# lh3/yak

Measured on AMD Instinct MI355X. Metric: distinct k-mers counted/sec (k=31), yak count -b37 two-pass protocol, .yak bit-exact, higher is better.
Workload: dtype u64

## Files before the change

### yak_amd/csrc/engine_ctx.cpp

```cpp
#include "engine_int.h"
#include <atomic>

static thread_local char g_err[512] = "";

extern "C" const char *yakamd_last_error(void) { return g_err; }
int yk_set_error(const char *fmt, ...) { va_list ap; va_start(ap, fmt); vsnprintf(g_err, sizeof(g_err), fmt, ap); va_end(ap); fprintf(stderr, "[E::yak_amd] %s\n", g_err); return -1; }

extern "C" int yakamd_device_count(void)
{
	int n = 0;
	if (hipGetDeviceCount(&n) != hipSuccess) return 0;
	int ok = 0;
	for (int i = 0; i < n; ++i) {
		hipDeviceProp_t pr;
		if (hipGetDeviceProperties(&pr, i) == hipSuccess && strncmp(pr.gcnArchName, "gfx950", 6) == 0) ++ok;
	}
	return ok;
}

extern "C" yakamd_ctx *yakamd_ctx_of(yak_ch_t *h) { return ctx_of(h); }

BloomView bloom_view(yakamd_ctx *c)
{
	BloomView b;
// ... 218 lines not shown
u64 yk_ctx_keys_total(yakamd_ctx *c) { return c->img_keys_total; }
void yk_ctx_range(yakamd_ctx *c, int *lo, int *hi) { *lo = c->plo; *hi = c->phi; }

struct yak_ht_t { uint32_t bits, count; uint32_t *used; uint64_t *keys; };

static std::atomic<int64_t> g_host_syncs{0};
extern "C" int64_t yakamd_host_syncs(void) { return g_host_syncs.load(); }

int yk_ctx_sync_host(yakamd_ctx *c, yak_ch_t *h)
{
	if (__atomic_load_n(&c->host_valid, __ATOMIC_ACQUIRE)) return 0;
	static std::mutex mu;
	std::lock_guard<std::mutex> lk(mu);
	if (c->host_valid) return 0;
	HIPCK(hipSetDevice(c->dev));
	++g_host_syncs;
	if (c->hm_slots < c->n_slots) {
		c->hm_keys.reset(); c->hm_used.reset(); c->hm_slots = 0;
		void *hk = 0, *hu = 0;
		HIPCK(hipHostMalloc(&hk, c->n_slots * 8));
		c->hm_keys.reset((u64*)hk);
		HIPCK(hipHostMalloc(&hu, c->n_slots / 8));
		c->hm_used.reset((u32*)hu);
		c->hm_slots = c->n_slots;
	}
	HIPCK(hipMemcpyAsync(c->hm_keys.get(), c->d_keys, c->n_slots * 8, hipMemcpyDeviceToHost, c->st));
	HIPCK(hipMemcpyAsync(c->hm_used.get(), c->d_used, c->n_slots / 8, hipMemcpyDeviceToHost, c->st));
	HIPCK(hipStreamSynchronize(c->st));
	if (!c->hts) c->hts.reset((yak_ht_t*)calloc(c->P, sizeof(yak_ht_t)));
	for (int p = 0; p < c->P; ++p) {
// ... 42 lines not shown
```

### yak_amd/csrc/engine_int.h

```cpp
#ifndef YK_ENGINE_INT_H
#define YK_ENGINE_INT_H
#include <stdio.h>
#include <stdlib.h>
#include <string.h>
#include <stdarg.h>
#include <vector>
#include <map>
#include <string>
#include <mutex>
#include <algorithm>
#include <memory>
#include "yk_device.h"
#include "tally.h"
#include "engine.h"
#include "dev_buf.h"

#define fail(...) yk_set_error(__VA_ARGS__)
#define HIPCK(x) do { hipError_t e_ = (x); if (e_ != hipSuccess) return fail("%s:%d: %s -> %s", __FILE__, __LINE__, #x, hipGetErrorString(e_)); } while (0)

static inline double now_ms() { return yk_now_ms(); }

static inline int64_t env_i64(const char *name, int64_t dflt) { return yk_knob(name, dflt); }

static inline int ceil_log2_u64(u64 x) { int b = 0; while ((1ull << b) < x) ++b; return b; }
// ... 26 lines not shown
struct HostFree { void operator()(void *p) const { (void)hipHostFree(p); } };
struct CFree { void operator()(void *p) const { free(p); } };
struct yak_ht_t;

struct Kept { DevBuf<Rec> own; Rec *d_rec = 0; u64 n = 0; u64 t0 = 0, span = 0; std::vector<u64> bstart; int fmt = 0; };

struct PassBufs {
	std::vector<Kept> kept; u64 kept_bytes = 0;
	AccTab acc = {}; DevBuf<AccSlot> acc_mem; u64 acc_count = 0;
	DevVec<Rec> rec;
	DevVec<uint8_t> hpc;
	DevVec<u64> newlist, miss, cand;
};

struct Retained { DevBuf<Rec> rec; u64 n = 0; std::vector<u64> bstart; };
struct Ret2 { DevBuf<Rec> r2; DevBuf<u64> sbstart, koff, kkc, segbase; DevBuf<u32> kc2; FastParams fp = {}; u64 n_total = 0, n_keys = 0; bool valid = false; };
struct RetainedInput { std::vector<Retained> l1; u64 l1_bytes = 0; Ret2 l2; };

struct yakamd_ctx {
	CtxStream st;
	int k = 0, pre = 0, P = 0, n_hash = 0, bf_shift = 0, nb = 0;
	bool has_bloom = false;
	int dev = 0, plo = 0, phi = 0;

	DevBuf<u32> d_bits, d_used, d_delta;
	DevBuf<u64> d_off, d_keys;
	u64 n_slots = 0;
	std::vector<u32> h_bits, h_count;
	std::vector<u64> h_off;
	u64 img_keys_total = 0;

	DevBuf<u32> d_bf; size_t bf_words = 0;
	bool bf_virgin = false;
	bool bf_deferred = false;
	DevBuf<u32> d_multi; int multi_bits = 0;

	bool delta_dirty = false;
	bool in_pass = false; int create_new = 0; bool bloom_mode = false; bool gate_off = false; int or_mode = 0;
	PassBufs pass;
	DevBuf<u64> d_counters, d_lastput, d_lpbatch;
	DevBuf<u32> d_missing, d_nmissing;
	DevVec<uint8_t> stage;
	bool hpc = false;
	DevVec<u32> rows; DevBuf<u64> d_partial, d_bstart; int nb_bits = 0;
	bool fast = false; u64 fast_budget = 0; u64 t_pass0 = 0; bool t_pass0_set = false; u64 keys_at_begin = 0;
// ... 11 lines not shown

	bool host_valid = false;
	std::unique_ptr<u64[], HostFree> hm_keys; std::unique_ptr<u32[], HostFree> hm_used; u64 hm_slots = 0;
	std::unique_ptr<yak_ht_t[], CFree> hts;
};

struct yak_ch_ext { yak_ch_t pub; yakamd_ctx *ctx; u32 magic; int n_sub; yak_ch_t **sub; };
#define EXT_MAGIC 0x59414b41u

static inline yakamd_ctx *ctx_of(const yak_ch_t *h)
{
	const yak_ch_ext *e = (const yak_ch_ext*)h;
	return (h && e->magic == EXT_MAGIC) ? e->ctx : 0;
}

static inline ImgView img_view(yakamd_ctx *c)
{
	ImgView v;
	v.bits = c->d_bits; v.off = c->d_off; v.keys = c->d_keys; v.used = c->d_used; v.delta = c->d_delta;
	v.pre = c->pre; v.k = c->k;
	return v;
}

struct ImageState { yakamd_ctx *c; bool sharded, in_pass; };
ImageState yk_image_state(const yak_ch_t *h);
yakamd_ctx *yk_whole_image_ctx(const yak_ch_t *h, int min_cnt, const char *what, const char *no_gpu, const char *even_k);

struct OutFile {
	FILE *f = 0;
	const char *name = "-";
	bool own = false;
	OutFile() = default;
	OutFile(const OutFile&) = delete;
	OutFile &operator=(const OutFile&) = delete;
	~OutFile() { if (own && f) fclose(f); }
	bool open(const char *fn) { own = fn && strcmp(fn, "-") != 0; if (own) name = fn; f = own ? fopen(fn, "wb") : stdout; return f != 0; }
// ... 37 lines not shown
```

### yak_amd/csrc/engine_pass.cpp

```cpp
#include "engine_int.h"
#include "seg_sort_tile.h"

static int acc_reserve(yakamd_ctx *c, u64 incoming)
{
	PassBufs &ps = c->pass;
	const u64 need = ps.acc_count + incoming;
	int want = std::max(c->pre + 2, ceil_log2_u64((u64)(need / 0.6) + 1));
	if (want < 12) want = 12;
	if (ps.acc.s && ps.acc.bits >= want) return 0;
	AccTab nt;
	DevBuf<AccSlot> mem;
	nt.bits = want; nt.pre = c->pre; nt.mask = (1ull << want) - 1;
	if (mem.alloc((size_t)1 << want)) return -1;
	nt.s = mem;
	yk_launch_acc_init(nt.s, 1ull << want, c->st);
	if (ps.acc.s) {
		yk_launch_acc_rehash(ps.acc, nt, c->st);
		HIPCK(hipStreamSynchronize(c->st));
	}
	ps.acc_mem = std::move(mem);
	ps.acc = nt;
	return 0;
}

// ... 192 lines not shown
		if (env_i64("YAKAMD_VERBOSE", 0)) fprintf(stderr, "[yak_amd] key-owning count: 2^%d slots per range (up to 2^%d ranges per sub-table), %u keys of LDS room, %zu B of LDS, %u boundary-crossing instances%s\n",
		                                          rng_log, rb, kmax, lds, xn[0], xn[1] ? " (list overflow: second sweep)" : "");
		if (hipStreamSynchronize(c->st) != hipSuccess) r = fail("count sweep failed");
	}
	return r;
}

int consume_records(yakamd_ctx *c, const Rec *d_rec, int64_t n_rec, u64 t0, u64 batch_lo, u64 batch_hi, const u64 *d_bstart, int hash_only, int ytag)
{
	if (n_rec <= 0) return 0;
	ImgView img = img_view(c);
	c->st_cur.n_instances += n_rec;
	if (batch_hi > c->t_end) c->t_end = batch_hi;
	if (!c->create_new) {
		c->delta_dirty = true;
		EvTimer tm(c->st);
		if (d_bstart) {
			const int r = count_own(c, d_rec, d_bstart, hash_only, ytag);
			if (r <= 0 || ytag) {
				insert_ms(c, tm);
				return r;
			}
		}
		const size_t lds = d_bstart ? count_lds_bytes(c) : 0;
		if (!lds && d_bstart && hash_only && c->nb_bits == c->pre && env_i64("YAKAMD_COUNT_RNG", 1) != 0) {
			const int r = count_by_ranges(c, d_rec, n_rec, d_bstart);
			if (r <= 0) {
				insert_ms(c, tm);
				return r;
			}
// ... 248 lines not shown
	const size_t NB = (size_t)1 << c->nb_bits;
	if (part_reserve(c, 1)) return -1;
	HIPCK(hipMemcpyAsync(c->d_bstart, h_bstart, (NB + 1) * 8, hipMemcpyHostToDevice, c->st));
	const int r = consume_records(c, (const Rec*)d_hash_u64, n, 0, 0, 0, c->d_bstart, 1);
	HIPCK(hipStreamSynchronize(c->st));
	return r;
}

extern "C" int yakamd_count_hashes_dev(yak_ch_t *h, const void *d_hash_u64, int64_t n)
{
	yakamd_ctx *c = ctx_of(h);
	if (!c || !c->in_pass || c->create_new) return fail("count_hashes needs an open create_new = 0 pass");
	HIPCK(hipSetDevice(c->dev));
	if (n <= 0) return 0;
	c->delta_dirty = true;
	EvTimer tm(c->st);
	yk_launch_img_count_h((const u64*)d_hash_u64, n, img_view(c), c->st);
	insert_ms(c, tm);
	c->st_cur.n_instances += n;
	return 0;
}

extern "C" int yakamd_retain_input(yak_ch_t *h, int on)
{
	yakamd_ctx *c = ctx_of(h);
	if (!c) return fail("not an engine table");
	if (c->in_pass) return fail("yakamd_retain_input inside a pass");
	HIPCK(hipSetDevice(c->dev));
	c->retain_on = on != 0;
	if (!on) retained_drop(c);
// ... 4 lines not shown
{
	yakamd_ctx *c = ctx_of(h);
	if (!c || c->retain_broken) return 0;
	u64 n = c->ret.l2.valid ? c->ret.l2.n_total : 0;
	for (auto &r : c->ret.l1) n += r.n;
	return (int64_t)n;
}

extern "C" int yakamd_count_retained(yak_ch_t *h)
{
	yakamd_ctx *c = ctx_of(h);
	if (!c || !c->in_pass || c->create_new) return fail("yakamd_count_retained needs an open create_new = 0 pass");
	HIPCK(hipSetDevice(c->dev));
	const Ret2 &l2 = c->ret.l2;
	if (l2.valid && !c->retain_broken && l2.kc2) {
		EvTimer tm(c->st);
		yk_launch_cnt2_apply(l2.fp, l2.kkc, l2.kc2, l2.segbase, img_view(c), c->st);
		const double ms = insert_ms(c, tm);
		const bool bad = hipGetLastError() != hipSuccess;
		c->st_cur.n_instances += (int64_t)l2.n_total;
		c->st_cur.pass2_path = 1; yk_event(YKE_PASS2_FUSED);
		if (env_i64("YAKAMD_VERBOSE", 0)) fprintf(stderr, "[yak_amd] count pass: the counts of the pass before applied (%llu keys, %.2f ms)\n", (unsigned long long)l2.n_keys, ms);
		retained_drop(c);
		return bad ? fail("applying the counts of the pass before failed") : 0;
	}
	if (l2.valid && !c->retain_broken) {
		DevBuf<u32> d_kcnt;
		if (d_kcnt.alloc(l2.n_keys)) return -1;
		HIPCK(hipMemsetAsync(c->d_nmissing, 0, 4, c->st));
		EvTimer tm(c->st);
		yk_launch_cnt2(l2.fp, l2.sbstart, l2.r2, l2.koff, l2.kkc, l2.segbase, d_kcnt, img_view(c), l2.n_keys, c->d_nmissing, c->st);
		u32 used = 1;
		(void)hipMemcpyAsync(&used, c->d_nmissing, 4, hipMemcpyDeviceToHost, c->st);
		const double ms = insert_ms(c, tm);
		if (used) c->delta_dirty = true;
		d_kcnt.reset();
		const bool bad = hipGetLastError() != hipSuccess;
// ... 127 lines not shown
```

### yak_amd/csrc/engine_slice.cpp

```cpp
#include "engine_int.h"
#include "seg_sort_tile.h"

void chunk_runs(ChunkTable &t, const void *base, size_t stride, const u64 *start, size_t n_buckets, u64 len)
{
	t.h.clear();
	t.first.assign(n_buckets + 1, 0);
	for (size_t q = 0; q < n_buckets; ++q) {
		t.first[q] = (u32)t.h.size();
		for (u64 o = start[q]; o < start[q + 1]; o += len) {
			Chunk2 ch = {};
			ch.rec = (const Rec*)((const char*)base + o * stride); ch.n = (u32)std::min<u64>(len, start[q + 1] - o); ch.bucket = (u32)q;
			t.h.push_back(ch);
		}
		if (t.h.size() > t.first[q]) t.h.back().spare = 1;
	}
	t.first[n_buckets] = (u32)t.h.size();
}


struct Slice {
	FastParams fp;
	u64 n_total = 0, sort_tmax = 0, budget = 0;
	int fmt_in = 0, s2 = 0, s2a = 0, s2b = 0;
	bool three = false, nowb_plan = false, keep2 = false;
// ... 376 lines not shown
	s.r2.reset(); s.ovf2.reset();
	if (slice_gather(c, s)) return -1;
	s.lo_kc.reset(); s.lo_T.reset(); s.lo_nsel.reset(); s.lo_lp.reset(); s.lo_nd.reset(); s.lo_c2.reset();
	s.kc2.reset(); s.sbstart.reset(); s.ndist.reset(); s.koff.reset();
	s.lap(c, "gather of the selected keys");
	if (slice_sort(c, s)) return -1;
	s.kc[s.cur ^ 1].reset(); s.tt[s.cur ^ 1].reset();
	s.lap(c, "sort by insertion time");
	{
		EvTimer tm(c->st);
		s.ro.resize(c->P);
		if (yk_run_replay(c, s.m, s.kc[s.cur], s.tt[s.cur], c->d_lastput, 0, false, &s.ro)) return -1;
		c->st_cur.ms_replay += tm.stop();
	}
	s.lap(c, "exact layout");
	return 0;
}

int fast_abandon(yakamd_ctx *c)
{
	for (auto &k : c->pass.kept) if (k.fmt) return fail("a batch was fed out of stream order after tagged 8-byte batches were kept: feed in order, or set YAKAMD_REC8=0");
	c->fast = false;
	yk_event(YKE_FAST_ABANDONED);
	c->retain_broken = true; retained_drop(c);
	int r = 0;
	for (auto &k : c->pass.kept) {
		if (!r) r = consume_records(c, k.d_rec, (int64_t)k.n, k.t0, k.t0, k.t0 + k.span);
		k.own.reset();
	}
	c->pass.kept.clear(); c->pass.kept_bytes = 0;
// ... 53 lines not shown
```

### yak_amd/csrc/engine_table.cpp

```cpp
#include "engine_int.h"

int yk_ctx_hist(yakamd_ctx *c, int64_t *cnt1024)
{
	HIPCK(hipSetDevice(c->dev));
	DevBuf<u64> d_h;
	if (d_h.alloc(1024)) return -1;
	HIPCK(hipMemsetAsync(d_h, 0, 1024 * 8, c->st));
	yk_launch_img_hist(img_view(c), c->n_slots, d_h, c->st);
	const hipError_t e = hipMemcpyAsync(cnt1024, d_h, 1024 * 8, hipMemcpyDeviceToHost, c->st);
	const hipError_t e2 = hipStreamSynchronize(c->st);
	return e == hipSuccess && e2 == hipSuccess ? 0 : fail("hist: %s", hipGetErrorString(e != hipSuccess ? e : e2));
}

int yk_ctx_setcnt(yakamd_ctx *c, int cnt)
{
	HIPCK(hipSetDevice(c->dev));
	yk_launch_img_setcnt(img_view(c), c->n_slots, (u32)cnt & 1023u, c->st);
	HIPCK(hipStreamSynchronize(c->st));
	c->host_valid = false;
	return 0;
}

int yk_ctx_clear(yakamd_ctx *c)
{
	HIPCK(hipSetDevice(c->dev));
	yk_launch_img_clear(img_view(c), c->n_slots, c->st);
	HIPCK(hipStreamSynchronize(c->st));
	c->host_valid = false;
	return 0;
}

static int rebuild(yakamd_ctx *c, int cmin, int cmax, int which, yakamd_ctx *other, u64 *tot)
{
	HIPCK(hipSetDevice(c->dev));
	const int P = c->P;
	if (other && (other->pre != c->pre || other->k != c->k)) return fail("tables of different k / prefix length");
	const ImgView ov = other ? img_view(other) : img_view(c);
	std::vector<u32> m(P), init(P);
	std::vector<u64> seg_off(P + 1, 0);
	DevBuf<u64> d_kc, d_segoff; DevBuf<u32> d_segcnt;
	const int RG = yk_shrink_shares();
	std::vector<u32> mr((size_t)P * RG);
	if (d_segcnt.alloc((size_t)P * RG) || d_segoff.alloc(P + 1)) return -1;
	yk_launch_shrink_count(img_view(c), P, cmin, cmax, which, ov, d_segcnt, c->st, 1);
// ... 11 lines not shown
	const int r = yk_run_replay(c, m, d_kc, 0, 0, &init, true);
	c->st_last.ms_shrink = tm.stop();
	if (r) return r;
	*tot = c->img_keys_total;
	return 0;
}

int yk_ctx_shrink(yakamd_ctx *c, int cmin, int cmax, u64 *tot) { return rebuild(c, cmin, cmax, 0, 0, tot); }
int yk_ctx_subtract(yakamd_ctx *c, yakamd_ctx *other, u64 *tot) { return rebuild(c, 0, 1023, 1, other, tot); }
int yk_ctx_isec(yakamd_ctx *c, yakamd_ctx *other, u64 *tot) { return rebuild(c, 0, 1023, 2, other, tot); }

#define YK_LEAVE 0xfffffffeu
static int resize_tables(yakamd_ctx *c, const std::vector<u32> &new_bits)
{
	HIPCK(hipSetDevice(c->dev));
	const int P = c->P;
	std::vector<ResizeTask> tasks(P);
	std::vector<u64> new_off(P);
	std::vector<u32> bits_after(P);
	u64 tot = 0;
	for (int p = 0; p < P; ++p) {
		ResizeTask &t = tasks[p];
		t.old_bits = c->h_bits[p]; t.old_off = c->h_off[p]; t.pad = 0;
		t.rehash = new_bits[p] != YK_LEAVE;
		t.new_bits = t.rehash ? new_bits[p] : c->h_bits[p];
		bits_after[p] = t.new_bits;
		const u64 n = t.old_bits == YK_NOCAP ? 0 : (u64)1 << t.old_bits, N = t.new_bits == YK_NOCAP ? 0 : (u64)1 << t.new_bits;
		t.new_off = new_off[p] = tot;
		tot += std::max<u64>(32, std::max(n, N));
	}
// ... 63 lines not shown
	HIPCK(hipStreamSynchronize(c->st));
	*d_hash = hash.release(); *d_t = t.release();
	if (d_cnt) *d_cnt = cnt.release();
	return 0;
}

int yk_ctx_add_counts(yakamd_ctx *c, const u64 *d_hash, const unsigned short *d_cnt, u64 n)
{
	if (c->in_pass) return fail("yk_ctx_add_counts during an open pass");
	if (n == 0) return 0;
	HIPCK(hipSetDevice(c->dev));
	DevBuf<u32> d_missing;
	u32 missing = 0;
	if (d_missing.alloc(1)) return -1;
	HIPCK(hipMemsetAsync(d_missing, 0, 4, c->st));
	yk_launch_img_add_counts(d_hash, d_cnt, n, img_view(c), c->plo, c->phi, d_missing, c->st);
	HIPCK(hipGetLastError());
	HIPCK(hipMemcpyAsync(&missing, d_missing, 4, hipMemcpyDeviceToHost, c->st));
	HIPCK(hipStreamSynchronize(c->st));
	c->host_valid = false;
	if (missing) return fail("sum: a listed key is not in the table after its create pass: the counts were not all added");
	return 0;
}

int yk_ctx_dump_image_dev(yakamd_ctx *c, int lo, int hi, u64 **d_img, u64 *n_words)
{
	HIPCK(hipSetDevice(c->dev));
	const int P = c->P, n = hi - lo;
	*d_img = 0; *n_words = 0;
	if (lo < 0 || hi > P || n <= 0) return fail("yk_ctx_dump_image_dev: sub-tables [%d, %d) of %d", lo, hi, P);
// ... 31 lines not shown
	const int P = c->P;
	std::vector<u32> m(P), init(P);
	u64 tot = 0;
	for (int p = 0; p < P; ++p) { m[p] = sizes[p]; init[p] = kh_bits_for(caps[p]); tot += sizes[p]; }
	DevBuf<u64> d_kc;
	if (d_kc.alloc(tot)) return -1;
	HIPCK(hipMemcpyAsync(d_kc, keys, tot * 8, hipMemcpyHostToDevice, c->st));
	return yk_run_replay(c, m, d_kc, 0, 0, &init, true);
}

int yk_ctx_inc(yakamd_ctx *c, u64 hash, int *count)
{
	if (c->in_pass) return fail("yak_ch_inc during an open pass");
	HIPCK(hipSetDevice(c->dev));
	u64 out[2];
	yk_launch_img_inc(img_view(c), hash, c->d_counters, c->st);
	HIPCK(hipMemcpyAsync(out, c->d_counters, 16, hipMemcpyDeviceToHost, c->st));
	HIPCK(hipStreamSynchronize(c->st));
	if (out[0] == ~0ull) { *count = -1; return 0; }
	*count = (int)out[1];
	if (c->host_valid && c->hm_keys) c->hm_keys[out[0]] = (c->hm_keys[out[0]] & ~1023ull) | out[1];
	return 0;
}
```

### yak_amd/csrc/kern_count.inc

```
__device__ __forceinline__ u32 sub_of(u64 h, const FastParams &fp)
{
	const u64 x = h >> fp.pre;
	if (fp.s2_bits == 0) return 0;
	return (u32)((x & ((1ull << fp.sw) - 1)) >> fp.ssh) & ((1u << fp.s2_bits) - 1);
}

__device__ __forceinline__ u32 r8_rank(const u64 *src_, int64_t i, u32 before, u32 n, u32 after)
{
	const u64 YK_GLOBAL *src = yk_global(u64, src_);
	const u64 me = src[i];
	const u32 tg = (u32)me & YK_R8_TOGGLE, pos = (u32)me & 1023u;
	int64_t a = i, e = i + 1;
	while (a > -(int64_t)before && ((u32)src[a - 1] & YK_R8_TOGGLE) == tg) --a;
	while (e < (int64_t)n + after && ((u32)src[e] & YK_R8_TOGGLE) == tg) ++e;
	u32 r = 0;
	for (int64_t j = a; j < e; ++j) r += ((u32)src[j] & 1023u) < pos;
	return (u32)((int64_t)before + a) + r;
}
template <bool NEED_T>
__device__ __forceinline__ void p2_load(const Chunk2 &c, u32 i, const FastParams &fp, u64 *h, u32 *t)
{
	if (c.pad == 1) {
		const u64 *src = (const u64*)c.rec;
		*h = (yk_global(u64, src)[i] >> YK_R8_TAG_BITS) << fp.pre | c.bucket;
// ... 902 lines not shown
		};
		if (lo + tid < hi) take(r0);
		if (lo + 256 + tid < hi) take(r1);
		if (lo + 512 + tid < hi) take(r2);
		for (u64 i = lo + 768 + tid; i < hi; i += 256) take(rec8[i]);
		__syncthreads();
		if (in_lds) {
			for (u32 i = tid; i < nk; i += 256) { const u32 s = s_slot[i]; key_cnt[ko + i] = s_C[s]; s_K[s] = YK_EMPTY; s_C[s] = 0; }
		} else for (u32 i = tid; i < nk; i += 256) key_cnt[ko + i] = 0;
		it = itn;
		__syncthreads();
	}
}

__global__ __launch_bounds__(256)
void k_cnt2_apply(const u64 *__restrict__ key_kc, const u32 *__restrict__ key_cnt, const u64 *__restrict__ seg_base, int plo, int pre, ImgView img)
{
	const u32 p = (u32)plo + blockIdx.y;
	const u64 a = seg_base[p], b = seg_base[p + 1];
	for (u64 i = a + (u64)blockIdx.x * 256 + threadIdx.x; i < b; i += (u64)gridDim.x * 256) {
		const u32 c = key_cnt[i];
		if (!c) continue;
		const u64 kid = key_kc[i] >> 10;
		const u32 bits = img.bits[p];
		if (bits == YK_NOCAP) continue;
		const u64 *keys = img.keys + img.off[p];
		const u32 nmask = (1u << bits) - 1;
		u32 s = yk_h2b((u32)kid, bits);
		const u32 first = s;
		for (;;) {
			const u64 kc = keys[s];
			if (kc == YK_EMPTY) break;
			if (kc >> 10 == kid) {
				const u64 n = (kc & 1023) + c;
				yk_global_rw(u64, img.keys)[img.off[p] + s] = (kc & ~1023ull) | (n > 1023 ? 1023 : n);
				break;
			}
			s = (s + 1) & nmask;
			if (s == first) break;
		}
	}
}

__global__ __launch_bounds__(256)
void k_nsel_scan(const u32 *__restrict__ nsel, int s2_bits, int plo, int phi, int P, const u64 *__restrict__ seg_base, u64 *__restrict__ key_off)
{
	__shared__ u32 s_w[5];
	const u32 p = blockIdx.x, S2 = 1u << s2_bits, tid = threadIdx.x, lane = tid & 63, wave = tid >> 6;
	const size_t b0 = (size_t)p * S2;
// ... 222 lines not shown
```

### yak_amd/csrc/kern_general.inc

```
__device__ __forceinline__ u64 acc_home(const AccTab &t, u64 key)
{
	const int rb = t.bits - t.pre;
	const u64 p = key & ((1ull << t.pre) - 1);
	const u64 r = ((key >> t.pre) * 0x9E3779B97F4A7C15ull) >> (64 - rb);
	return p << rb | r;
}

__device__ __forceinline__ AccSlot *acc_claim(const AccTab &t, u64 key, bool *created)
{
	u64 i = acc_home(t, key);
	*created = false;
	for (;;) {
		AccSlot *s = t.s + i;
		u64 cur = s->key;
		if (cur == key) return s;
		if (cur == YK_EMPTY) {
			cur = atomicCAS(&s->key, YK_EMPTY, key);
			if (cur == YK_EMPTY) { *created = true; return s; }
			if (cur == key) return s;
		}
		i = (i + 1) & t.mask;
	}
}

// ... 213 lines not shown
	for (u64 i = (u64)blockIdx.x * blockDim.x + threadIdx.x; i < n_slots; i += stride)
		if (img.used[i >> 5] >> (i & 31) & 1) atomicAdd(&s_h[img.keys[i] & 1023u], 1u);
	__syncthreads();
	for (u32 i = threadIdx.x; i < 1024; i += 256) if (s_h[i]) atomicAdd(&hist[i], (unsigned long long)s_h[i]);
}

__global__ __launch_bounds__(256)
void k_img_setcnt(ImgView img, u64 n_slots, u32 cnt)
{
	const u64 stride = (u64)gridDim.x * blockDim.x;
	for (u64 i = (u64)blockIdx.x * blockDim.x + threadIdx.x; i < n_slots; i += stride)
		if (img.used[i >> 5] >> (i & 31) & 1) img.keys[i] = (img.keys[i] & ~1023ull) | cnt;
}

__global__ __launch_bounds__(256)
void k_img_clear(ImgView img, u64 n_slots)
{
	const u64 stride = (u64)gridDim.x * blockDim.x;
	for (u64 i = (u64)blockIdx.x * blockDim.x + threadIdx.x; i < n_slots; i += stride)
		if (img.used[i >> 5] >> (i & 31) & 1) img.keys[i] &= ~1023ull;
}

#define AC_THREADS 256
#define AC_U 2
template <bool LONG>
__global__ __launch_bounds__(AC_THREADS)
void k_img_add_counts(const u64 *__restrict__ hash, const unsigned short *__restrict__ cnt, u64 n, ImgView img, int plo, int phi, int tab, u32 *missing)
{
	extern __shared__ __attribute__((aligned(16))) u64 s_ac[];
	const u32 pmask = (1u << img.pre) - 1;
	if (tab) {
		for (u32 p = threadIdx.x; p <= pmask; p += AC_THREADS) { const u32 b = img.bits[p]; s_ac[p] = img.off[p] | (u64)(b == YK_NOCAP ? 63u : b) << 58; }
		__syncthreads();
	}
	const u64 YK_GLOBAL *ghash = yk_global(u64, hash);
// ... 310 lines not shown
```

### yak_amd/csrc/kern_launch.inc

```
#include <atomic>
struct DevOnce {
	std::atomic<unsigned> m{0};
	static unsigned bit() { int d = 0; (void)hipGetDevice(&d); return 1u << (d & 31); }
	bool operator!() const { return !(m.load(std::memory_order_acquire) & bit()); }
	DevOnce &operator=(bool) { m.fetch_or(bit(), std::memory_order_release); return *this; }
};
extern "C" {

void yk_launch_extract(const uint8_t *bases, int64_t pos0, int64_t n, int64_t t_sub, int k, int pre, int plo, int phi,
                       u64 *out_hash, u32 *out_t, u64 *cursor, hipStream_t st)
{
	if (n <= pos0) return;
	const u64 tiles = ((u64)(n - pos0) + XT_TILE - 1) / XT_TILE;
	YK_LAUNCH(k_extract, dim3((unsigned)tiles), dim3(XT_THREADS), 0, st, bases, pos0, n, t_sub, k, pre, plo, phi, out_hash, out_t, cursor);
}

__global__ __launch_bounds__(256)
void k_pack(const uint8_t *__restrict__ a, int64_t n, u32 *__restrict__ codes, u32 *__restrict__ valid)
{
	const int64_t w = (int64_t)blockIdx.x * 256 + threadIdx.x, p0 = w * 32;
	if (p0 >= n) return;
	u32 c0 = 0, c1 = 0, v = 0;
	for (int j = 0; j < 32; ++j) {
		const int64_t p = p0 + j;
// ... 133 lines not shown
}

void yk_launch_img_count_h(const u64 *hash, int64_t n, ImgView img, hipStream_t st)
{
	if (n <= 0) return;
	YK_LAUNCH(k_img_count_h, dim3(grid_for((u64)n)), dim3(256), 0, st, hash, n, img);
}

void yk_launch_img_inc(ImgView img, u64 hash, u64 *out2, hipStream_t st) { YK_LAUNCH(k_img_inc, dim3(1), dim3(1), 0, st, img, hash, out2); }

void yk_launch_img_fold(ImgView img, u64 n_slots, hipStream_t st)
{
	if (n_slots) YK_LAUNCH(k_img_fold, dim3(grid_for(n_slots)), dim3(256), 0, st, img, n_slots);
}

void yk_launch_img_clear(ImgView img, u64 n_slots, hipStream_t st)
{
	if (n_slots) YK_LAUNCH(k_img_clear, dim3(grid_for(n_slots)), dim3(256), 0, st, img, n_slots);
}

void yk_launch_img_hist(ImgView img, u64 n_slots, u64 *hist, hipStream_t st)
{
	if (n_slots) YK_LAUNCH(k_img_hist, dim3(grid_for(n_slots)), dim3(256), 0, st, img, n_slots, (unsigned long long*)hist);
}

void yk_launch_img_setcnt(ImgView img, u64 n_slots, u32 cnt, hipStream_t st)
{
	if (n_slots) YK_LAUNCH(k_img_setcnt, dim3(grid_for(n_slots)), dim3(256), 0, st, img, n_slots, cnt);
}

void yk_launch_lastput(const Rec *rec, int64_t n, u64 t0, u64 t_from, AccTab tab, ImgView img,
                       int img_nonempty, int bloom_mode, const u32 *only_missing, u64 *lp_batch, hipStream_t st)
{
// ... 408 lines not shown
                              u64 *dst_kc, u64 *dst_t, int shift, u32 *dig_hist, int n_dig, hipStream_t st, int big)
{
	if (big) YK_LAUNCH((k_seg_sort_pass<8, 1024>), dim3(P), dim3(1024), 0, st, seg_base, seg_cnt, src_kc, src_t, dst_kc, dst_t, shift, dig_hist, n_dig);
	else YK_LAUNCH((k_seg_sort_pass<8, 256>), dim3(P), dim3(256), 0, st, seg_base, seg_cnt, src_kc, src_t, dst_kc, dst_t, shift, dig_hist, n_dig);
}
void yk_launch_cnt2(FastParams fp, const u64 *sbstart, const Rec *rec, const u64 *key_off, const u64 *key_kc, const u64 *seg_base, u32 *key_cnt, ImgView img, u64 n_keys, u32 *used_delta, hipStream_t st)
{
	const u32 n_sb = (u32)(fp.phi - fp.plo) << fp.s2_bits;
	const int wgs = (int)yk_knob("YAKAMD_CNT2_WGS", 256 * 1024);
	const int small_max = (int)yk_knob("YAKAMD_CNT2_SMALL", 128);
	const dim3 grid(std::min<u32>(n_sb, (u32)std::max(1, wgs)));
	if (n_sb && small_max >= 0 && n_keys / n_sb <= (u64)small_max) YK_LAUNCH((k_cnt2<512, 320>), grid, dim3(256), 0, st, fp, sbstart, rec, key_off, key_kc, img, n_sb, key_cnt, used_delta);
	else YK_LAUNCH((k_cnt2<2048, 1280>), grid, dim3(256), 0, st, fp, sbstart, rec, key_off, key_kc, img, n_sb, key_cnt, used_delta);
	yk_launch_cnt2_apply(fp, key_kc, key_cnt, seg_base, img, st);
}
void yk_launch_cnt2_apply(FastParams fp, const u64 *key_kc, const u32 *key_cnt, const u64 *seg_base, ImgView img, hipStream_t st)
{
	const int n_p = fp.phi - fp.plo;
	const int per = std::max(1, 8192 / std::max(1, n_p));
	YK_LAUNCH(k_cnt2_apply, dim3(per, n_p), dim3(256), 0, st, key_kc, key_cnt, seg_base, fp.plo, fp.pre, img);
}
void yk_launch_nsel_scan(const u32 *nsel, int s2_bits, int plo, int phi, int P, const u64 *seg_base, u64 *key_off, hipStream_t st)
{
	YK_LAUNCH(k_nsel_scan, dim3(P), dim3(256), 0, st, nsel, s2_bits, plo, phi, P, seg_base, key_off);
}

static int cu_count()
{
	int dev = 0, n_cu = 0;
	return hipGetDevice(&dev) == hipSuccess && hipDeviceGetAttribute(&n_cu, hipDeviceAttributeMultiprocessorCount, dev) == hipSuccess && n_cu >= 1 ? n_cu : 256;
}

int yk_launch_inspect(const u64 *keys, const u64 *off, u64 n, int n_sub, int sub_lo, int hdr, int pre_a, int has_b, ImgView img, int blo, int bhi,
                      int ref, u64 *J, hipStream_t st)
{
// ... 120 lines not shown
```

### yak_amd/csrc/layout.cpp

```cpp
#include "engine_int.h"


static void legacy_replay_launch(yakamd_ctx *c, const std::vector<ReplayTask> &tasks, const ReplayTask *d_tasks, u64 *nk, u32 *nu, u32 *su, u32 *so, u64 *sp,
                                 const u64 *d_rec_kc, const u64 *d_rec_t, const u64 *d_lastput, u32 *d_ob, u32 *d_oc)
{
	const int P = c->P, n_active = c->phi - c->plo;
	u32 cap_top = 0;
	for (int p = 0; p < P; ++p) if (tasks[p].m) cap_top = std::max(cap_top, 1u << tasks[p].cap_max_bits);
	u32 lds_words = std::min<u32>(cap_top, (u32)env_i64("YAKAMD_REPLAY_LDS", 16384));
	int n_thr = n_active <= 256 ? 1024 : n_active <= 512 ? 512 : 256;
	if (lds_words * 4 >= 96 * 1024) n_thr = 1024; else if (lds_words * 4 >= 48 * 1024) n_thr = std::max(n_thr, 512);
	n_thr = (int)env_i64("YAKAMD_REPLAY_THREADS", n_thr);
	yk_launch_replay(d_tasks, P, n_thr, c->d_keys, c->d_used, nk, nu, su, so, sp, d_rec_kc, d_rec_t, d_lastput, d_ob, d_oc, lds_words, c->st);
}

int yk_image_commit(yakamd_ctx *c, DevBuf<u64> &&keys, DevBuf<u32> &&used, u64 tot, const std::vector<u64> &new_off)
{
	c->d_keys = std::move(keys); c->d_used = std::move(used); c->d_delta.reset();
	c->n_slots = tot;
	c->h_off = new_off;
	HIPCK(hipMemcpyAsync(c->d_bits, c->h_bits.data(), c->P * 4, hipMemcpyHostToDevice, c->st));
	HIPCK(hipMemcpyAsync(c->d_off, c->h_off.data(), c->P * 8, hipMemcpyHostToDevice, c->st));
	HIPCK(hipStreamSynchronize(c->st));
	c->img_keys_total = 0;
	for (int p = 0; p < c->P; ++p) c->img_keys_total += c->h_count[p];
	c->host_valid = false;
	return 0;
}

static u32 g_r2_used = 0, g_r2_refused = 0;

struct Replay2 {
	yakamd_ctx *c;
// ... 168 lines not shown
	if (env_i64("YAKAMD_REPLAY2", 1) == 0 || in.P > 65536) return 1;
	Replay2 s;
	s.c = c; s.d_rec_kc = d_rec_kc; s.d_rec_t = d_rec_t; s.d_lastput = d_lastput;
	int r;
	if ((r = r2_plan(s, in)) != 0) return r;
	if ((r = r2_small_part(s)) != 0) return r;
	if ((r = r2_buffers(s)) != 0) return r;
	r2_steps(s);
	return r2_publish_commit(s);
}

int yk_run_replay(yakamd_ctx *c, const std::vector<u32> &m, const u64 *d_rec_kc, const u64 *d_rec_t,
                  const u64 *d_lastput, const std::vector<u32> *init_bits, bool from_empty, const std::vector<u64> *rec_off)
{
	const int P = c->P;
	const ReplayIn in = { P, c->h_bits.data(), c->h_count.data(), c->h_off.data(), m.data(), init_bits ? init_bits->data() : 0, rec_off ? rec_off->data() : 0, from_empty, d_lastput != 0 };
	{
		const int r2 = run_replay_v2(c, in, d_rec_kc, d_rec_t, d_lastput);
		if (r2 <= 0) return r2;
	}
	ReplayPlan pl;
	pl.classify(in, ReplayPlan::SB_NONE, (u32)env_i64("YAKAMD_DBG", 0));
	const u64 tot = pl.tot;
	DevBuf<u32> nu; DevBuf<u64> nk; DevBuf<u32> d_oc, d_ob; DevBuf<ReplayTask> d_tasks; DevBuf<u64> sp; DevBuf<u32> so, su;
	const bool par = env_i64("YAKAMD_PAR_REPLAY", 1) != 0;
	if ((par && sp.alloc(2 * tot)) || nk.alloc(tot) || nu.alloc(tot / 32) || su.alloc(tot / 32) || so.alloc(tot) ||
	    d_tasks.alloc(P) || d_ob.alloc(P) || d_oc.alloc(P)) return -1;
	HIPCK(hipMemsetAsync(nk, 0xff, tot * 8, c->st));
	HIPCK(hipMemsetAsync(nu, 0, tot / 8, c->st));
	HIPCK(hipMemcpyAsync(d_tasks, pl.tasks.data(), P * sizeof(ReplayTask), hipMemcpyHostToDevice, c->st));
// ... 16 lines not shown
```

### yak_amd/csrc/yk_device.h

```cpp
#ifndef YK_DEVICE_H
#define YK_DEVICE_H

#include <stdint.h>
#include <hip/hip_runtime.h>
#include "replay_plan.h"

typedef ulonglong2 Rec;

#define YK_EMPTY   0xFFFFFFFFFFFFFFFFull
#define YK_TINF    0xFFFFFFFFFFFFFFFFull
#define YK_FLAG_FP 1u

__host__ __device__ static inline u64 yk_hash64_inv(u64 x, u64 m)
{
	u64 t;
	t = x - (x << 31); x = (x - (t << 31)) & m;
	t = x ^ x >> 28; x = x ^ t >> 28;
	x = (x * 14933078535860113213ULL) & m;
	t = x ^ x >> 14; t = x ^ t >> 14; t = x ^ t >> 14; x = x ^ t >> 14;
	x = (x * 15244667743933553977ULL) & m;
	t = x ^ x >> 24; x = x ^ t >> 24;
	t = ~x; t = ~(x - (t << 21)); t = ~(x - (t << 21)); x = ~(x - (t << 21)) & m;
	return x;
}
// ... 93 lines not shown
                     u32 *tile_cnt, const u64 *tile_off, void *list, hipStream_t st);
u64 yk_graph_tile(void);
int yk_launch_graph(int what, int inflight, int grid_want, const u64 *tile0, const u64 *key0, uint8_t *edges, u32 *wrank, u64 *tally, u64 t_lo, u64 t_hi, u64 n_slots,
                    int P, int min_cnt, void *out, u64 out_key0, u64 out_n, ImgView img, hipStream_t st);
int64_t yk_hpc_tile(int packed);
int64_t yk_hpc_tiles(int packed, int64_t n);
void yk_launch_hpc_count(const void *in, const u32 *valid, int64_t n, u32 *tcnt, hipStream_t st);
void yk_launch_hpc_scatter(const void *in, const u32 *valid, int64_t n, const u64 *toff, uint8_t *out, hipStream_t st);
void yk_launch_hpc_remap(const uint8_t *a, int64_t n, const u64 *toff, const u64 *off, const u32 *len, int64_t n_seq, u64 *off_out, u32 *len_out, hipStream_t st);
int yk_launch_img_count_lds(const void *rec, int hash_only, const u64 *bstart, ImgView img, int plo, int phi, size_t lds, u64 *compact, u32 stride, hipStream_t st);
void yk_launch_img_count_h(const u64 *hash, int64_t n, ImgView img, hipStream_t st);
void yk_launch_img_inc(ImgView img, u64 hash, u64 *out2, hipStream_t st);
void yk_launch_img_fold(ImgView img, u64 n_slots, hipStream_t st);
void yk_launch_img_hist(ImgView img, u64 n_slots, u64 *hist, hipStream_t st);
void yk_launch_img_setcnt(ImgView img, u64 n_slots, u32 cnt, hipStream_t st);
void yk_launch_img_clear(ImgView img, u64 n_slots, hipStream_t st);
void yk_launch_lastput(const Rec *rec, int64_t n, u64 t0, u64 t_from, AccTab tab, ImgView img,
                       int img_nonempty, int bloom_mode, const u32 *only_missing, u64 *lp_batch, hipStream_t st);
void yk_launch_lastput_merge(u64 *lastput, const u64 *lp_batch, u32 *missing, u32 *n_missing, int P, int plo, int phi, hipStream_t st);

void yk_launch_bf_test(AccTab tab, const u64 *newlist, u64 n_new, BloomView bf, u64 *miss, hipStream_t st);
void yk_launch_bf_set(AccTab tab, const u64 *newlist, u64 n_new, BloomView bf, const u64 *miss,
                      u32 *multi, int multi_bits, u64 *counters, hipStream_t st);
void yk_launch_bf_check(AccTab tab, const u64 *newlist, u64 n_new, BloomView bf, const u64 *miss,
                        const u32 *multi, int multi_bits, u64 *cand, u64 *counters, hipStream_t st);
void yk_launch_bf_mapfill(AccTab tab, const u64 *newlist, u64 n_new, BloomView bf, const u64 *miss,
                          const u32 *multi, int multi_bits, u64 *map, int map_bits, hipStream_t st);
void yk_launch_bf_resolve(AccTab tab, const u64 *newlist, const u64 *cand, u64 n_cand, BloomView bf,
                          const u64 *miss, const u64 *map, int map_bits, hipStream_t st);

void yk_launch_select_count(AccTab tab, int bloom_mode, int P, u32 *seg_cnt, hipStream_t st);
// ... 81 lines not shown
int yk_launch_img_count_own(const void *rec, int hash_only, int cross, int ytag, const u64 *bstart, ImgView img, int plo, int phi, int rb, int rng_log, u32 kmax,
                            size_t lds, u64 *list, u32 *list_n, u32 list_cap, hipStream_t st);
int yk_lc2_ok(FastParams fp);
int yk_lc2_per_sb(int bloom_mode);
void yk_launch_lc2(FastParams fp, const u64 *sbstart, const Rec *rec, u32 *bloom32, ImgView img, LcOut O, u64 *counters, u32 *ovf_list, hipStream_t st);
void yk_launch_lc_sum(const u32 *nsel, int s2_bits, int plo, int phi, u32 *seg_cnt, hipStream_t st);
void yk_launch_lc_compact(LcOut O, const u64 *sbstart, int s2_bits, int plo, int phi, u64 t_pass0, const u64 *seg_base,
                          u64 *out_kc, u64 *out_T, u64 *lastput, u32 *ndist_p, Rec *out_kt, u32 *out_c2, hipStream_t st);
void yk_launch_part2_ts(const Chunk2 *chunks, int n_chunks, const u32 *chunk_first, const u64 *bbase, FastParams fp, int P, u32 *rows2, u64 *sbstart, Rec *out, hipStream_t st);
int yk_launch_ts_rank(const u64 *binstart, const Rec *in, int w, int j, u32 bin_lo, u32 n_bins, u64 *out_kc, u64 *out_t, u32 *fail, hipStream_t st);
void yk_launch_kt_split(const Rec *in, u64 n, u64 *out_kc, u64 *out_t, hipStream_t st);
void yk_launch_bf_rebuild(FastParams fp, const u64 *sbstart, const Rec *rec, u32 *bloom32, hipStream_t st);
void yk_launch_lc_sum3(LcOut O, int s2_bits, int plo, int phi, u64 t_pass0, u32 *seg_cnt, u64 *lastput, u32 *ndist_p, hipStream_t st);
void yk_launch_lc_gather(LcOut O, const u64 *sbstart, const u64 *key_off, int s2_bits, int plo, int phi, u64 *out_kc, u64 *out_T, Rec *out_kt, u32 *out_c2, hipStream_t st);
void yk_launch_cnt2(FastParams fp, const u64 *sbstart, const Rec *rec, const u64 *key_off, const u64 *key_kc, const u64 *seg_base, u32 *key_cnt, ImgView img, u64 n_keys, u32 *used_delta, hipStream_t st);
void yk_launch_cnt2_apply(FastParams fp, const u64 *key_kc, const u32 *key_cnt, const u64 *seg_base, ImgView img, hipStream_t st);
void yk_launch_nsel_scan(const u32 *nsel, int s2_bits, int plo, int phi, int P, const u64 *seg_base, u64 *key_off, hipStream_t st);
void yk_launch_seg_sort_pass2(const u64 *seg_base, const u32 *seg_cnt, int P, const u64 *src_kc, const u64 *src_t,
                              u64 *dst_kc, u64 *dst_t, int shift, u32 *dig_hist, int n_dig, hipStream_t st, int big);
#ifdef __cplusplus
}
#endif
enum { YKC_NOVF2 = 7 };

#endif
```

Before: 1.093 billion.

## Defer image clear and fold it into pass-two count application

Clearing the count image no longer launches a kernel and synchronizes immediately. It sets a pending flag that is settled lazily before any image access. When pass two applies retained counts to a whole image built in pass one, the clear is turned into a bump sweep (each used slot's count incremented by one). The apply kernel then writes only the keys whose final count differs from that guess. This removes a blocking clear and sync and most of the scattered hash-table writes in the apply step, at the cost of extra state tracking and correctness conditions around when the whole-image shortcut is valid.

```diff
diff --git a/yak_amd/csrc/engine_ctx.cpp b/yak_amd/csrc/engine_ctx.cpp
--- a/yak_amd/csrc/engine_ctx.cpp
+++ b/yak_amd/csrc/engine_ctx.cpp
@@ -256,6 +256,7 @@
 	std::lock_guard<std::mutex> lk(mu);
 	if (c->host_valid) return 0;
 	HIPCK(hipSetDevice(c->dev));
+	if (yk_image_settle(c)) return -1;
 	++g_host_syncs;
 	if (c->hm_slots < c->n_slots) {
 		c->hm_keys.reset(); c->hm_used.reset(); c->hm_slots = 0;
diff --git a/yak_amd/csrc/engine_int.h b/yak_amd/csrc/engine_int.h
--- a/yak_amd/csrc/engine_int.h
+++ b/yak_amd/csrc/engine_int.h
@@ -8,6 +8,7 @@
 #include <map>
 #include <string>
 #include <mutex>
+#include <atomic>
 #include <algorithm>
 #include <memory>
 #include "yk_device.h"
@@ -64,7 +65,10 @@
 };
 
 struct Retained { DevBuf<Rec> rec; u64 n = 0; std::vector<u64> bstart; };
-struct Ret2 { DevBuf<Rec> r2; DevBuf<u64> sbstart, koff, kkc, segbase; DevBuf<u32> kc2; FastParams fp = {}; u64 n_total = 0, n_keys = 0; bool valid = false; };
+struct Ret2 {
+	DevBuf<Rec> r2; DevBuf<u64> sbstart, koff, kkc, segbase; DevBuf<u32> kc2; FastParams fp = {}; u64 n_total = 0, n_keys = 0; bool valid = false;
+	bool whole_image = false;
+};
 struct RetainedInput { std::vector<Retained> l1; u64 l1_bytes = 0; Ret2 l2; };
 
 struct yakamd_ctx {
@@ -79,6 +83,7 @@
 	std::vector<u32> h_bits, h_count;
 	std::vector<u64> h_off;
 	u64 img_keys_total = 0;
+	std::atomic<bool> clear_pending{false};
 
 	DevBuf<u32> d_bf; size_t bf_words = 0;
 	bool bf_virgin = false;
@@ -120,12 +125,20 @@
 	return (h && e->magic == EXT_MAGIC) ? e->ctx : 0;
 }
 
-static inline ImgView img_view(yakamd_ctx *c)
+int yk_image_settle(yakamd_ctx *c);
+static inline void yk_image_touched(yakamd_ctx *c) { c->ret.l2.whole_image = false; }
+
+static inline ImgView img_view_pending(yakamd_ctx *c)
 {
 	ImgView v;
 	v.bits = c->d_bits; v.off = c->d_off; v.keys = c->d_keys; v.used = c->d_used; v.delta = c->d_delta;
 	v.pre = c->pre; v.k = c->k;
 	return v;
+}
+static inline ImgView img_view(yakamd_ctx *c)
+{
+	if (c->clear_pending) (void)yk_image_settle(c);
+	return img_view_pending(c);
 }
 
 struct ImageState { yakamd_ctx *c; bool sharded, in_pass; };
diff --git a/yak_amd/csrc/engine_pass.cpp b/yak_amd/csrc/engine_pass.cpp
--- a/yak_amd/csrc/engine_pass.cpp
+++ b/yak_amd/csrc/engine_pass.cpp
@@ -230,6 +230,7 @@
 	if (batch_hi > c->t_end) c->t_end = batch_hi;
 	if (!c->create_new) {
 		c->delta_dirty = true;
+		yk_image_touched(c);
 		EvTimer tm(c->st);
 		if (d_bstart) {
 			const int r = count_own(c, d_rec, d_bstart, hash_only, ytag);
@@ -508,6 +509,7 @@
 	HIPCK(hipSetDevice(c->dev));
 	if (n <= 0) return 0;
 	c->delta_dirty = true;
+	yk_image_touched(c);
 	EvTimer tm(c->st);
 	yk_launch_img_count_h((const u64*)d_hash_u64, n, img_view(c), c->st);
 	insert_ms(c, tm);
@@ -542,13 +544,19 @@
 	HIPCK(hipSetDevice(c->dev));
 	const Ret2 &l2 = c->ret.l2;
 	if (l2.valid && !c->retain_broken && l2.kc2) {
+		const bool bump = c->clear_pending && l2.whole_image && env_i64("YAKAMD_PASS2_BUMP", 1) != 0;
+		const ImgView img = bump ? img_view_pending(c) : img_view(c);
 		EvTimer tm(c->st);
-		yk_launch_cnt2_apply(l2.fp, l2.kkc, l2.kc2, l2.segbase, img_view(c), c->st);
+		if (bump) {
+			c->clear_pending = false;
+			yk_launch_img_clear(img, c->n_slots, c->st, 1);
+		}
+		yk_launch_cnt2_apply(l2.fp, l2.kkc, l2.kc2, l2.segbase, img, c->st, bump);
 		const double ms = insert_ms(c, tm);
 		const bool bad = hipGetLastError() != hipSuccess;
 		c->st_cur.n_instances += (int64_t)l2.n_total;
 		c->st_cur.pass2_path = 1; yk_event(YKE_PASS2_FUSED);
-		if (env_i64("YAKAMD_VERBOSE", 0)) fprintf(stderr, "[yak_amd] count pass: the counts of the pass before applied (%llu keys, %.2f ms)\n", (unsigned long long)l2.n_keys, ms);
+		if (env_i64("YAKAMD_VERBOSE", 0)) fprintf(stderr, "[yak_amd] count pass: the counts of the pass before applied (%llu keys, %.2f ms%s)\n", (unsigned long long)l2.n_keys, ms, bump ? "; with the pending clear, in one sweep" : "");
 		retained_drop(c);
 		return bad ? fail("applying the counts of the pass before failed") : 0;
 	}
diff --git a/yak_amd/csrc/engine_slice.cpp b/yak_amd/csrc/engine_slice.cpp
--- a/yak_amd/csrc/engine_slice.cpp
+++ b/yak_amd/csrc/engine_slice.cpp
@@ -414,6 +414,9 @@
 		c->st_cur.ms_replay += tm.stop();
 	}
 	s.lap(c, "exact layout");
+	Ret2 &l2 = c->ret.l2;
+	l2.whole_image = s.keep2 && l2.valid && l2.kc2 && last && c->n_slices == 0 && c->keys_at_begin == 0 && !s.fp.img_nonempty && !c->retain_broken &&
+	                 l2.n_keys == c->img_keys_total;
 	return 0;
 }
 
diff --git a/yak_amd/csrc/engine_table.cpp b/yak_amd/csrc/engine_table.cpp
--- a/yak_amd/csrc/engine_table.cpp
+++ b/yak_amd/csrc/engine_table.cpp
@@ -18,16 +18,30 @@
 	yk_launch_img_setcnt(img_view(c), c->n_slots, (u32)cnt & 1023u, c->st);
 	HIPCK(hipStreamSynchronize(c->st));
 	c->host_valid = false;
+	yk_image_touched(c);
 	return 0;
 }
 
 int yk_ctx_clear(yakamd_ctx *c)
 {
-	HIPCK(hipSetDevice(c->dev));
-	yk_launch_img_clear(img_view(c), c->n_slots, c->st);
-	HIPCK(hipStreamSynchronize(c->st));
+	c->clear_pending = true;
 	c->host_valid = false;
 	return 0;
+}
+
+int yk_image_settle(yakamd_ctx *c)
+{
+	static std::mutex mu;
+	std::lock_guard<std::mutex> lk(mu);
+	if (!c->clear_pending) return 0;
+	int cur = c->dev;
+	(void)hipGetDevice(&cur);
+	if (cur != c->dev) HIPCK(hipSetDevice(c->dev));
+	yk_launch_img_clear(img_view_pending(c), c->n_slots, c->st);
+	const hipError_t e = hipStreamSynchronize(c->st);
+	c->clear_pending = false;
+	if (cur != c->dev) (void)hipSetDevice(cur);
+	return e == hipSuccess ? 0 : fail("clear: %s", hipGetErrorString(e));
 }
 
 static int rebuild(yakamd_ctx *c, int cmin, int cmax, int which, yakamd_ctx *other, u64 *tot)
@@ -69,6 +83,7 @@
 static int resize_tables(yakamd_ctx *c, const std::vector<u32> &new_bits)
 {
 	HIPCK(hipSetDevice(c->dev));
+	if (yk_image_settle(c)) return -1;
 	const int P = c->P;
 	std::vector<ResizeTask> tasks(P);
 	std::vector<u64> new_off(P);
@@ -162,6 +177,7 @@
 	u32 missing = 0;
 	if (d_missing.alloc(1)) return -1;
 	HIPCK(hipMemsetAsync(d_missing, 0, 4, c->st));
+	yk_image_touched(c);
 	yk_launch_img_add_counts(d_hash, d_cnt, n, img_view(c), c->plo, c->phi, d_missing, c->st);
 	HIPCK(hipGetLastError());
 	HIPCK(hipMemcpyAsync(&missing, d_missing, 4, hipMemcpyDeviceToHost, c->st));
@@ -223,6 +239,7 @@
 	if (c->in_pass) return fail("yak_ch_inc during an open pass");
 	HIPCK(hipSetDevice(c->dev));
 	u64 out[2];
+	yk_image_touched(c);
 	yk_launch_img_inc(img_view(c), hash, c->d_counters, c->st);
 	HIPCK(hipMemcpyAsync(out, c->d_counters, 16, hipMemcpyDeviceToHost, c->st));
 	HIPCK(hipStreamSynchronize(c->st));
diff --git a/yak_amd/csrc/kern_count.inc b/yak_amd/csrc/kern_count.inc
--- a/yak_amd/csrc/kern_count.inc
+++ b/yak_amd/csrc/kern_count.inc
@@ -940,13 +940,16 @@
 }
 
 __global__ __launch_bounds__(256)
-void k_cnt2_apply(const u64 *__restrict__ key_kc, const u32 *__restrict__ key_cnt, const u64 *__restrict__ seg_base, int plo, int pre, ImgView img)
+void k_cnt2_apply(const u64 *__restrict__ key_kc, const u32 *__restrict__ key_cnt, const u64 *__restrict__ seg_base, int plo, int pre, ImgView img, int fix)
 {
 	const u32 p = (u32)plo + blockIdx.y;
 	const u64 a = seg_base[p], b = seg_base[p + 1];
 	for (u64 i = a + (u64)blockIdx.x * 256 + threadIdx.x; i < b; i += (u64)gridDim.x * 256) {
 		const u32 c = key_cnt[i];
-		if (!c) continue;
+		if (fix) {
+			const u32 c1 = (u32)key_kc[i] & 1023u;
+			if (c == (c1 < 1023u ? c1 + 1 : 1023u)) continue;
+		} else if (!c) continue;
 		const u64 kid = key_kc[i] >> 10;
 		const u32 bits = img.bits[p];
 		if (bits == YK_NOCAP) continue;
@@ -958,7 +961,7 @@
 			const u64 kc = keys[s];
 			if (kc == YK_EMPTY) break;
 			if (kc >> 10 == kid) {
-				const u64 n = (kc & 1023) + c;
+				const u64 n = fix ? c : (kc & 1023) + c;
 				yk_global_rw(u64, img.keys)[img.off[p] + s] = (kc & ~1023ull) | (n > 1023 ? 1023 : n);
 				break;
 			}
diff --git a/yak_amd/csrc/kern_general.inc b/yak_amd/csrc/kern_general.inc
--- a/yak_amd/csrc/kern_general.inc
+++ b/yak_amd/csrc/kern_general.inc
@@ -251,11 +251,14 @@
 }
 
 __global__ __launch_bounds__(256)
-void k_img_clear(ImgView img, u64 n_slots)
+void k_img_clear(ImgView img, u64 n_slots, int bump)
 {
 	const u64 stride = (u64)gridDim.x * blockDim.x;
 	for (u64 i = (u64)blockIdx.x * blockDim.x + threadIdx.x; i < n_slots; i += stride)
-		if (img.used[i >> 5] >> (i & 31) & 1) img.keys[i] &= ~1023ull;
+		if (img.used[i >> 5] >> (i & 31) & 1) {
+			const u64 kc = img.keys[i];
+			img.keys[i] = !bump ? kc & ~1023ull : (kc & 1023) < 1023 ? kc + 1 : kc;
+		}
 }
 
 #define AC_THREADS 256
diff --git a/yak_amd/csrc/kern_launch.inc b/yak_amd/csrc/kern_launch.inc
--- a/yak_amd/csrc/kern_launch.inc
+++ b/yak_amd/csrc/kern_launch.inc
@@ -171,9 +171,9 @@
 	if (n_slots) YK_LAUNCH(k_img_fold, dim3(grid_for(n_slots)), dim3(256), 0, st, img, n_slots);
 }
 
-void yk_launch_img_clear(ImgView img, u64 n_slots, hipStream_t st)
-{
-	if (n_slots) YK_LAUNCH(k_img_clear, dim3(grid_for(n_slots)), dim3(256), 0, st, img, n_slots);
+void yk_launch_img_clear(ImgView img, u64 n_slots, hipStream_t st, int bump)
+{
+	if (n_slots) YK_LAUNCH(k_img_clear, dim3(grid_for(n_slots)), dim3(256), 0, st, img, n_slots, bump);
 }
 
 void yk_launch_img_hist(ImgView img, u64 n_slots, u64 *hist, hipStream_t st)
@@ -612,11 +612,11 @@
 	else YK_LAUNCH((k_cnt2<2048, 1280>), grid, dim3(256), 0, st, fp, sbstart, rec, key_off, key_kc, img, n_sb, key_cnt, used_delta);
 	yk_launch_cnt2_apply(fp, key_kc, key_cnt, seg_base, img, st);
 }
-void yk_launch_cnt2_apply(FastParams fp, const u64 *key_kc, const u32 *key_cnt, const u64 *seg_base, ImgView img, hipStream_t st)
+void yk_launch_cnt2_apply(FastParams fp, const u64 *key_kc, const u32 *key_cnt, const u64 *seg_base, ImgView img, hipStream_t st, int fix)
 {
 	const int n_p = fp.phi - fp.plo;
 	const int per = std::max(1, 8192 / std::max(1, n_p));
-	YK_LAUNCH(k_cnt2_apply, dim3(per, n_p), dim3(256), 0, st, key_kc, key_cnt, seg_base, fp.plo, fp.pre, img);
+	YK_LAUNCH(k_cnt2_apply, dim3(per, n_p), dim3(256), 0, st, key_kc, key_cnt, seg_base, fp.plo, fp.pre, img, fix);
 }
 void yk_launch_nsel_scan(const u32 *nsel, int s2_bits, int plo, int phi, int P, const u64 *seg_base, u64 *key_off, hipStream_t st)
 {
diff --git a/yak_amd/csrc/layout.cpp b/yak_amd/csrc/layout.cpp
--- a/yak_amd/csrc/layout.cpp
+++ b/yak_amd/csrc/layout.cpp
@@ -17,6 +17,7 @@
 int yk_image_commit(yakamd_ctx *c, DevBuf<u64> &&keys, DevBuf<u32> &&used, u64 tot, const std::vector<u64> &new_off)
 {
 	c->d_keys = std::move(keys); c->d_used = std::move(used); c->d_delta.reset();
+	yk_image_touched(c);
 	c->n_slots = tot;
 	c->h_off = new_off;
 	HIPCK(hipMemcpyAsync(c->d_bits, c->h_bits.data(), c->P * 4, hipMemcpyHostToDevice, c->st));
@@ -215,6 +216,7 @@
                   const u64 *d_lastput, const std::vector<u32> *init_bits, bool from_empty, const std::vector<u64> *rec_off)
 {
 	const int P = c->P;
+	if (yk_image_settle(c)) return -1;
 	const ReplayIn in = { P, c->h_bits.data(), c->h_count.data(), c->h_off.data(), m.data(), init_bits ? init_bits->data() : 0, rec_off ? rec_off->data() : 0, from_empty, d_lastput != 0 };
 	{
 		const int r2 = run_replay_v2(c, in, d_rec_kc, d_rec_t, d_lastput);
diff --git a/yak_amd/csrc/yk_device.h b/yak_amd/csrc/yk_device.h
--- a/yak_amd/csrc/yk_device.h
+++ b/yak_amd/csrc/yk_device.h
@@ -131,7 +131,7 @@
 void yk_launch_img_fold(ImgView img, u64 n_slots, hipStream_t st);
 void yk_launch_img_hist(ImgView img, u64 n_slots, u64 *hist, hipStream_t st);
 void yk_launch_img_setcnt(ImgView img, u64 n_slots, u32 cnt, hipStream_t st);
-void yk_launch_img_clear(ImgView img, u64 n_slots, hipStream_t st);
+void yk_launch_img_clear(ImgView img, u64 n_slots, hipStream_t st, int bump = 0);
 void yk_launch_lastput(const Rec *rec, int64_t n, u64 t0, u64 t_from, AccTab tab, ImgView img,
                        int img_nonempty, int bloom_mode, const u32 *only_missing, u64 *lp_batch, hipStream_t st);
 void yk_launch_lastput_merge(u64 *lastput, const u64 *lp_batch, u32 *missing, u32 *n_missing, int P, int plo, int phi, hipStream_t st);
@@ -243,7 +243,7 @@
 void yk_launch_lc_sum3(LcOut O, int s2_bits, int plo, int phi, u64 t_pass0, u32 *seg_cnt, u64 *lastput, u32 *ndist_p, hipStream_t st);
 void yk_launch_lc_gather(LcOut O, const u64 *sbstart, const u64 *key_off, int s2_bits, int plo, int phi, u64 *out_kc, u64 *out_T, Rec *out_kt, u32 *out_c2, hipStream_t st);
 void yk_launch_cnt2(FastParams fp, const u64 *sbstart, const Rec *rec, const u64 *key_off, const u64 *key_kc, const u64 *seg_base, u32 *key_cnt, ImgView img, u64 n_keys, u32 *used_delta, hipStream_t st);
-void yk_launch_cnt2_apply(FastParams fp, const u64 *key_kc, const u32 *key_cnt, const u64 *seg_base, ImgView img, hipStream_t st);
+void yk_launch_cnt2_apply(FastParams fp, const u64 *key_kc, const u32 *key_cnt, const u64 *seg_base, ImgView img, hipStream_t st, int fix = 0);
 void yk_launch_nsel_scan(const u32 *nsel, int s2_bits, int plo, int phi, int P, const u64 *seg_base, u64 *key_off, hipStream_t st);
 void yk_launch_seg_sort_pass2(const u64 *seg_base, const u32 *seg_cnt, int P, const u64 *src_kc, const u64 *src_t,
                               u64 *dst_kc, u64 *dst_t, int shift, u32 *dig_hist, int n_dig, hipStream_t st, int big);
```

Result: faster. 1.139 billion, median of 6 (+4.2%).
